# NLESC-JCER/Fortran_Davidson

Measured on AMD Instinct MI355X. Metric: Davidson iterations/sec (dense DPR solve, matrix resident in HBM) + A*V HBM GB/s vs roofline, higher is better.
Workload: dtype f64

## Files before the change

fortran_davidson_amd/csrc/engine.hip:

```cpp
#include "engine_internal.h"

thread_local std::string g_err;
int fail(const std::string& msg) {
  g_err = msg;
  return 1;
}

int bind(E* e) {
  e->h0_take = e->h0_cols;
  e->h0_cols = 0;
  HIPCHK(hipSetDevice(e->device));
  return 0;
}

int collect_events(E* e) {
  e->ev_open = 0;
  for (int i = 0; i < e->ev_used; ++i) {
    if (!e->ev_done[i]) continue;
    HIPCHK(hipEventSynchronize(e->ev[i][1]));
    float ms = 0;
    HIPCHK(hipEventElapsedTime(&ms, e->ev[i][0], e->ev[i][1]));
    if (e->ev_kind[i] == 0) {
      e->st.apply_ms += ms;
      e->st.apply_bytes += e->ev_bytes[i];
// ... 147 lines not shown

Tune tune_from_env() {
  Tune t;
  auto geti = [](const char* name, int dflt) { const char* ev = getenv(name); return ev && *ev ? atoi(ev) : dflt; };
  t.sym_wide = geti("DAV_SYM_WIDE", t.sym_wide);
  t.sym_wide32 = geti("DAV_SYM_WIDE32", t.sym_wide32);
  t.sym_pair = geti("DAV_SYM_PAIR", t.sym_pair);
  t.sym_quad = geti("DAV_SYM_QUAD", t.sym_quad);
  t.sym_overlap = geti("DAV_SYM_OVERLAP", t.sym_overlap);
  t.sym_r = geti("DAV_SYM_R", t.sym_r);
  t.sym_tall = geti("DAV_SYM_TALL", t.sym_tall);
  t.sym_gen_wide = geti("DAV_SYM_GEN_WIDE", 1);
  t.sym_run = std::max(0, geti("DAV_SYM_RUN", 0));
  t.sym_run9 = std::max(0, geti("DAV_SYM_RUN9", 0));
  t.sym_mfma4 = geti("DAV_SYM_MFMA4", t.sym_mfma4);
  t.mv_target = std::max(0, geti("DAV_MV_TARGET", 0));
  t.mv_nsplit = std::max(0, geti("DAV_MV_NSPLIT", 0));
  t.b_resident = geti("DAV_B_RESIDENT", t.b_resident);
  t.coll_direct = geti("DAV_COLL_DIRECT", t.coll_direct);
  t.pg_pin = geti("DAV_PG_PIN", t.pg_pin);
  t.gram_wgs = geti("DAV_GRAM_WGS", t.gram_wgs);
  gram_set_fuse_chunks(geti("DAV_GRAM_FUSE", 0));
  t.gjd_trace = getenv("DAV_GJD_TRACE") != nullptr;
  t.harness_libm = geti("DAV_HARNESS_LIBM", 0);
  t.no_h0 = geti("DAV_NO_H0", 0);
  t.cheb_fuse = geti("DAV_CHEB_FUSE", t.cheb_fuse);
  t.coll_select = geti("DAV_COLL_SELECT", 1);
  t.coll_trial_corrupt = geti("DAV_COLL_TRIAL_CORRUPT", 0);
  t.coll_forced = getenv("DAV_SYM_OVERLAP") != nullptr || getenv("DAV_COLL_DIRECT") != nullptr;
  return t;
// ... 263 lines not shown
    e->sm[i].host = (double*)(e->arena_host + off_smh[i]);
    HIPCHK(hipEventCreateWithFlags(&e->sm[i].done, hipEventDisableTiming));
  }
  lt.lap("carve");
  for (int i = 0; i < N_EVPAIRS; ++i) {
    HIPCHK(hipEventCreate(&e->ev[i][0]));
    HIPCHK(hipEventCreate(&e->ev[i][1]));
  }
  lt.lap("events");
  HIPCHK(hipStreamSynchronize(e->stream));
  lt.lap("memset_sync");
  lt.print("dav_create");
  return 0;
}

extern "C" int dav_destroy(dav_handle_t e) {
  if (!e) return 0;
  LapTimer lt;
  hipSetDevice(e->device);
  if (e->stream) hipStreamSynchronize(e->stream);
  if (e->comm_stream) hipStreamSynchronize(e->comm_stream);
  lt.lap("sync");
  if (e->comm && g_rccl.lib) g_rccl.CommDestroy(e->comm);
  lt.lap("comm");
  pool_begin_of_destroy();
  if (e->arena) pool_free(e->arena);
  if (e->arena_host) pool_host_free(e->arena_host);
  lt.lap("arenas");
  pool_free(e->gjd_ws);
  pool_free(e->cheb_ws);
  ingest_release(e);
  shm_release(e);
  pool_free(e->sym_slab);
  pool_free(e->rr_H); pool_free(e->rr_S); pool_free(e->rr_Y); pool_free(e->rr_theta); pool_free(e->rr_work); pool_free(e->rr_info);
  pool_free(e->rr_Ypk); pool_free(e->rr_Y2pk); pool_free(e->rr_thpk);
  lt.lap("ingest_shm_slab_rr");
  for (int i = 0; i < 2; ++i) {
    if (e->ov_packed[i]) hipEventDestroy(e->ov_packed[i]);
    if (e->ov_gathered[i]) hipEventDestroy(e->ov_gathered[i]);
    if (e->ov_reduced[i]) hipEventDestroy(e->ov_reduced[i]);
    if (e->ov_scattered[i]) hipEventDestroy(e->ov_scattered[i]);
    pool_free(e->sym_wpart2[i]);
    pool_free(e->sym_wrecv2[i]);
  }
  if (e->comm_stream) hipStreamDestroy(e->comm_stream);
  if (e->wd) {
    { std::lock_guard<std::mutex> lk(e->wd->mu); e->wd->stop = true; }
    e->wd->cv.notify_all();
    e->wd->th.join();
    for (Watchdog::Lane& l : e->wd->lane) { if (l.check.ev) hipEventDestroy(l.check.ev); if (l.latest.ev) hipEventDestroy(l.latest.ev); }
    delete e->wd;
    e->wd = nullptr;
  }
  lt.lap("overlap_watchdog");
  sym_set_release(e->sym);
  lt.lap("sym_set");
  pool_free(e->sym_wpart);
  pool_free(e->coll_stage);
  pool_free(e->cb_x);
  pool_free(e->sym_wrecv);
// ... 134 lines not shown
```

fortran_davidson_amd/csrc/engine_apply.hip:

```cpp
#include "engine_internal.h"

bool inner_f32_tiles(E* e, OpDesc& o) {
  if (e->inner_bits != 32 || o.kind != DAV_KIND_DENSE || o.storage != 1 || o.a32_refused) return false;
  if (o.a32_valid) return true;
  const size_t count = (size_t)std::max<int64_t>(e->sym.ntiles, 1) * SYM_TB * SYM_TB;
  if (!o.a32 && pool_malloc(&o.a32, sizeof(float) * count) != hipSuccess) {
    (void)hipGetLastError();
    o.a32 = nullptr;
    o.a32_refused = true;
    return false;
  }
  launch_tiles_to_f32(e->stream, o.a, o.a32, (int64_t)count);
  o.a32_valid = true;
  return true;
}

static double* sym_slab_t(const E* e, const SymLaunch& L) { return e->sym_slab + (int64_t)L.ngroups * L.dstride; }
static void sym_sweep(E* e, const SymLaunch& L, const OpDesc& o, const SymSet& set, const double* xt) {
  if (L.nitems == 0) return;
  const SymPlan* pl = L.plan;
  const void* tiles = L.use32 ? (const void*)o.a32 : (const void*)o.a;
  double *slabD = e->sym_slab, *slabT = sym_slab_t(e, L);
  const int64_t xs = e->xt_group_stride, ds = L.dstride, ts = L.tstride;
  switch (L.family) {
    case SYM_ROW_STORED:
      return launch_matvec_sym(e->stream, o.a, set.row_off, set.items, set.nitems, xt, L.kk, slabD, slabT, L.ngroups, xs, ds, ts);
    case SYM_ROW_GENERATED:
      return launch_matvec_sym_generated(e->stream, op_params(o), e->n, set.items, set.nitems, xt, L.kk, slabD, slabT, L.ngroups, xs, ds, ts);
    case SYM_SUPER:
      return launch_matvec_sym9(e->stream, L.R, o.kind != DAV_KIND_DENSE, tiles, L.use32, set.row_off, o.kind != DAV_KIND_DENSE ? op_params(o) : OpParams{},
                                e->n, e->sym_nb, pl->items, pl->nitems, pl->zslot_begin, xt, L.kk, slabD, slabT, L.nwg, xs, ds, ts, e->tune.sym_mfma4 != 0);
    case SYM_WIDE:
    case SYM_WIDE_F32:
      return launch_matvec_symw(e->stream, L.nbw, L.tall, L.use32, tiles, set.row_off, e->sym_nb, pl->items, pl->nitems, pl->zslot_begin, xt, L.kk, slabD, slabT, L.nwg, xs, ds, ts);
    case SYM_WIDE_GENERATED:
// ... 2 lines not shown
}

static void count_apply(E* e, int which, int kk) { if (which == DAV_OP_A) { e->st.applies += 1; e->st.apply_cols += kk; } }

static int pack_operand(E* e, const double* src, int kk, bool gather) {
  launch_pack_xt(e->stream, src, e->ldp, e->nloc, e->nslab, kk, e->xt, e->xt_group_stride, e->row0);
  if (!gather) return 0;
  const int ngroups = (kk + 15) / 16;
  CollGroup grp(e);
  CHK(grp.begin(5, 8.0 * (double)e->nslab * 16 * ngroups * e->nranks));
  for (int g = 0; g < ngroups; ++g)
    CHK(coll_allgather(e, e->xt + g * e->xt_group_stride + e->row0 * 16, e->xt + g * e->xt_group_stride, (size_t)e->nslab * 16));
  return grp.end("all-gather of the new block", e->stream);
}

static void sym_reduce_groups(E* e, const SymLaunch& L, const SymSet& set, const int64_t* owned, double* out, int64_t chunk_rows, bool accumulate) {
  const int64_t total_rows = (int64_t)e->nranks * e->nslab;
  const double* slabT = sym_slab_t(e, L);
  for (int g = 0; g < L.ngroups; ++g) {
    const int kg = std::min(16, L.kk - 16 * g);
    const double *d = e->sym_slab + g * L.dstride, *t = slabT + g * L.tstride;
    double* og = out + (size_t)g * 16 * (size_t)(chunk_rows ? total_rows : e->ldp);
    if (L.plan)
      launch_sym9_reduce(e->stream, d, t, L.plan->row_begin, L.plan->zslot_begin, owned, L.plan->next_owned, L.R, e->sym_nb, e->nloc, kg, og, e->ldp,
                         chunk_rows, total_rows, accumulate);
    else
      launch_sym_reduce(e->stream, d, t, set.row_begin, owned, e->sym_nb, e->nloc, kg, og, e->ldp, chunk_rows, total_rows, accumulate);
  }
}

static int ensure_sym_wpart(E* e) {
  if (e->sym_wpart) return 0;
  HIPCHK(pool_malloc(&e->sym_wpart, sizeof(double) * (size_t)e->nranks * (size_t)e->nslab * 64));
  HIPCHK(pool_malloc(&e->sym_wrecv, sizeof(double) * (size_t)e->nslab * 64));
  return 0;
}

static int sym_scatter_to_panel(E* e, int kk, double* dst, bool accumulate, const char* what, double* h0 = nullptr, size_t h0_count = 0) {
  const size_t wstride = (size_t)e->nranks * (size_t)e->nslab * 16, rstride = (size_t)e->nslab * 16;
  const int ngroups = (kk + 15) / 16;
  CollGroup grp(e);
  CHK(grp.begin(6, 8.0 * (double)e->nslab * kk * e->nranks));
  for (int g = 0; g < ngroups; ++g)
// ... 242 lines not shown
                                     "-column launch on rank " + std::to_string(e->rank) + " (DAV_SYM_QUAD=0 / DAV_SYM_PAIR=0 on every rank select narrower launches)");
      if (L.ngroups > 2) { e->sym_no_quad = true; step = 32; kk = 32; }
      else { e->sym_no_pair = true; step = 16; kk = 16; }
      L = sym_launch(e, o, set, kk, use32, L.R);
    }
    int slot = -1, kslot = -1;
    if (timed) CHK(timed_begin(e, which == DAV_OP_A ? 0 : 2, sym_stored_bytes(e, o, set, partial, use32) + 16.0 * (double)e->n * kk, &slot));
    CHK(pack_operand(e, src + (int64_t)c * e->ldp, kk, multi));
    if (timed && which == DAV_OP_A) CHK(timed_begin(e, 4, 2.0 * (double)e->n * (double)e->n * kk / e->nranks, &kslot));
    if (timed && which == DAV_OP_B) {
      const double tiles_entries = (double)set.ntiles * SYM_TB * SYM_TB;
      if (stored) CHK(timed_begin(e, 8, (use32 ? 4.0 : 8.0) * tiles_entries + 16.0 * (double)e->n * kk, &kslot));
      else CHK(timed_begin(e, 9, tiles_entries * L.gen_evals, &kslot));
      if (kslot >= 0) e->ev_flops[kslot] = 4.0 * tiles_entries * kk;
    }
    sym_sweep(e, L, o, set, e->xt);
    CHK(timed_end(e, kslot));
    sym_reduce_groups(e, L, set, owned, multi ? e->sym_wpart : dst + (int64_t)c * e->ldp, multi ? e->nslab : 0, accumulate && !multi);
    if (multi) CHK(sym_scatter_to_panel(e, kk, dst + (int64_t)c * e->ldp, accumulate, "reduce-scatter of the partial products"));
    CHK(timed_end(e, slot));
    count_apply(e, which, kk);
  }
  HIPCHK(hipGetLastError());
  return 0;
}

static void sparse_traffic(const E* e, const OpDesc& o, int k, double* bytes, double* flops) {
  const double bb = (double)o.sp.b * o.sp.b, nnz = (double)o.sp.nnz;
  *bytes = 8.0 * bb * nnz + 4.0 * nnz + 8.0 * (double)(o.sp.nrows + 1) + 8.0 * (double)e->n * k + 8.0 * (double)e->nloc * k;
  *flops = 2.0 * bb * nnz * k;
}

static int apply_identity(E* e, const double* src, int k, double* dst) { launch_copy_columns(e->stream, src, e->ldp, dst, e->ldp, e->nloc_pad, k); return 0; }
// ... 275 lines not shown
```

fortran_davidson_amd/csrc/engine_internal.h:

```cpp
#pragma once
#include "davidson_hip_private.h"
#include "kernels.h"
#include "ingest.h"

#include <dlfcn.h>
#include <fcntl.h>
#include <pthread.h>
#include <sys/mman.h>
#include <sys/stat.h>
#include <unistd.h>
#include <rccl/rccl.h>

#include <algorithm>
#include <chrono>
#include <condition_variable>
#include <ctime>
#include <mutex>
#include <cmath>
#include <cstdio>
#include <cstring>
#include <numeric>
#include <string>
#include <thread>
#include <vector>
// ... 45 lines not shown
  const char* (*GetErrorString)(ncclResult_t) = nullptr;
  ncclResult_t (*CommCount)(const ncclComm_t, int*) = nullptr;
};
extern Rccl g_rccl;
int rccl_load();
#define NCCLCHK(call)                                                                              \
  do {                                                                                             \
    ncclResult_t r_ = (call);                                                                      \
    if (r_ != ncclSuccess) return fail(std::string(#call) + " failed: " + g_rccl.GetErrorString(r_)); \
  } while (0)

struct LocalGroup;
struct ShmGroup;

struct SymPlan {
  int R = 0, nitems = 0, nsuper = 0;
  int64_t zslots = 0;
  int* items = nullptr;
  int* row_begin = nullptr;
  int* zslot_begin = nullptr;
  int* next_owned = nullptr;
};
struct SymSet {
  std::vector<int64_t> row_off_h;
  int64_t* row_off = nullptr;
  int64_t ntiles = 0;
  int nitems = 0;
  int* items = nullptr;
  int* row_begin = nullptr;
  SymPlan plan[2];
  bool built = false;
};
void sym_set_release(SymSet& s);
enum SymFamily { SYM_ROW_STORED, SYM_ROW_GENERATED, SYM_SUPER, SYM_WIDE, SYM_WIDE_GENERATED, SYM_WIDE_F32 };
struct SymLaunch {
  SymFamily family = SYM_SUPER;
  int kk = 0, ngroups = 0;
  int R = 0, nwg = 0, nbw = 1;
  bool use32 = false, tall = false;
  const SymPlan* plan = nullptr;
  int nitems = 0;
  int64_t dstride = 0, tstride = 0;
  int gen_evals = 0;
};

struct SparseStore {
  int64_t* rp = nullptr;
  int32_t* col = nullptr;
  double* val = nullptr;
  CsrItem* items = nullptr;
  CsrLong* longs = nullptr;
  double* part = nullptr;
  int nitems = 0, nlong = 0;
  int64_t nnz = 0;
  int64_t nrows = 0;
  int b = 0;
  int64_t grow0 = 0;
  uint64_t* src = nullptr;
// ... 57 lines not shown
  int sym_run = 0;
  int sym_run9 = 0;
  int sym_mfma4 = 1;
  int64_t mv_target = 0;
  int64_t mv_nsplit = 0;
  int gram_wgs = 0;
  int pg_pin = 1;
  int coll_direct = 0;
  int b_resident = 1;
  bool gjd_trace = false;
  int coll_select = 1;
  int coll_trial_corrupt = 0;
  bool coll_forced = false;
  int no_h0 = 0;
  int harness_libm = 0;
  int cheb_fuse = 1;
};
Tune tune_from_env();

enum { COLL_PATH_UNDECIDED = -1, COLL_PATH_PROGRAM_ORDER = 0, COLL_PATH_DIRECT = 1, COLL_PATH_SECOND_STREAM = 2 };
struct CollTrial {
  bool ran = false;
  int selected = COLL_PATH_PROGRAM_ORDER, columns = 0;
  double ms[3] = {0, 0, 0}, ms_max[3] = {0, 0, 0};
  bool valid[3] = {true, false, false}, valid_all[3] = {true, false, false};
  double differing[3] = {0, 0, 0}, maxdiff[3] = {0, 0, 0};
  std::string message[3];
};

enum { GUESS_NONE = 0, GUESS_ONE_SHOT = 1, GUESS_RESULT = 2 };
// ... 45 lines not shown
  std::vector<double> agree_words;
  std::vector<double> agreed_inputs;
  double* agree_pin = nullptr;
  double* h0_dev = nullptr;
  double* cb_x = nullptr;
  size_t cb_x_doubles = 0;
  double* h0_host = nullptr;
  int h0_cap = 0, h0_cols = 0, h0_take = 0;
  int h0_kind[2] = {0, 0};
  hipStream_t comm_stream = nullptr;
  bool ov_ready = false;
  hipEvent_t ov_packed[2] = {nullptr, nullptr}, ov_gathered[2] = {nullptr, nullptr}, ov_reduced[2] = {nullptr, nullptr},
             ov_scattered[2] = {nullptr, nullptr};
  double* sym_wpart2[2] = {nullptr, nullptr};
  double* sym_wrecv2[2] = {nullptr, nullptr};
  bool rr_on = false;
  int64_t rr_ld = 0;
  double *rr_H = nullptr, *rr_S = nullptr, *rr_Y = nullptr, *rr_theta = nullptr, *rr_work = nullptr, *rr_info = nullptr;
  double *rr_Ypk = nullptr, *rr_Y2pk = nullptr, *rr_thpk = nullptr;
  int64_t rr_tp = 4;
  SmallBuf sm[N_SMALL];
  size_t small_doubles = 0;
  ncclComm_t comm = nullptr;
  int comm_ranks = 0;
  LocalGroup* lg = nullptr;
  ShmGroup* shm = nullptr;
  OpDesc op[2];
  int keep_map[2] = {0, 0};
  std::vector<double> diag_host[2];
  std::vector<int64_t> basis_order;
// ... 42 lines not shown
  bool image = false;
};

int bind(E* e);
int collect_events(E* e);
int timed_begin(E* e, int kind, double bytes, int* slot);
int timed_end(E* e, int slot);
int timed_begin_on(E* e, int kind, double bytes, int* slot, hipStream_t stream);
int timed_end_on(E* e, int slot, hipStream_t stream);
int small_upload(E* e, int i, const double* src, int64_t ld, int p, int q, int64_t* ldm_out);
int small_upload_multi(E* e, int i, SmallMat* mats, int n);
int small_upload_image(E* e, int i, const double* src, int64_t ld, int p, int q, int64_t* tp_out);
double* panel_ptr(E* e, int panel, int col);
int check_panel(E* e, int panel, int c0, int k);
int create_impl(E* e, int device, int64_t n, int max_cols, int gev, int rank, int nranks);
double wall_seconds();
void watchdog_loop(Watchdog* w);
bool has_comm(E* e);
int need_comm(E* e);
bool has_test_transport(const E* e);
size_t test_transport_max_message(const E* e);
int test_allgather(E* e, const double* send, double* recv, size_t count);
int test_allreduce(E* e, double* buf, size_t count);
int test_reduce_scatter(E* e, const double* send, double* recv, size_t count);
void shm_release(E* e);
int watch_mark(E* e, const char* what, hipStream_t stream);
int coll_group_begin(E* e);
int coll_group_end(E* e, const char* what, hipStream_t stream);
void coll_group_abort(E* e);
struct CollGroup {
// ... 66 lines not shown
```

fortran_davidson_amd/csrc/engine_operators.hip:

```cpp
#include "engine_internal.h"

int refresh_diag_host(E* e, int which) {
  if (which == DAV_OP_A) e->basis_order.clear();
  std::vector<double>& d = e->diag_host[which];
  d.assign((size_t)e->n, 0.0);
  if (!has_comm(e)) {
    CHK(need_comm(e));
    HIPCHK(hipMemcpyAsync(d.data(), e->op[which].diag, sizeof(double) * e->n, hipMemcpyDeviceToHost, e->stream));
    HIPCHK(hipStreamSynchronize(e->stream));
  } else {
    CHK(coll_allgather(e, e->op[which].diag, e->gather_dev, (size_t)e->nslab));
    HIPCHK(hipMemcpyAsync(d.data(), e->gather_dev, sizeof(double) * e->n, hipMemcpyDeviceToHost, e->stream));
    HIPCHK(hipStreamSynchronize(e->stream));
  }
  return 0;
}

static bool sym_wide_enabled(const E* e) { return e->tune.sym_wide > 1; }

static int sym_schedule(const E* e, int kk, bool stored_fp64) {
  const int forced = e->tune.sym_r;
  const int nb = (int)(e->ncols_pad / SYM_TB);
  int R = nb >= 200 ? (kk <= 8 ? 4 : 2) : (nb >= 64 && stored_fp64 ? 2 : 1);
  const bool tall = stored_fp64 && kk > 8 && kk <= 16 && nb >= 200 && sym_wide_enabled(e) && e->tune.sym_tall != 0;
// ... 20 lines not shown
    L.dstride = (int64_t)set.nitems * 16 * SYM_TB;
    L.tstride = (int64_t)e->sym_nb * (e->sym_nb - 1) / 2 * 16 * SYM_TB;
  } else {
    L.plan = &set.plan[R == 4 ? 1 : 0];
    L.nitems = L.plan->nitems;
    L.dstride = (int64_t)L.nitems * R * 16 * SYM_TB;
    L.tstride = L.plan->zslots * 16 * SYM_TB;
    if (stored && !use32 && wide > 0 && ((R == 2 && (kk > 16 || wide > 1)) || (R == 4 && kk > 8 && kk <= 16))) {
      L.family = SYM_WIDE; L.nbw = kk > 16 ? 2 : 1; L.tall = R == 4;
    } else if (generated_polynomial(o) && R == 2 && kk > 16 && wide > 0 && e->tune.sym_gen_wide) {
      L.family = SYM_WIDE_GENERATED; L.nbw = 2;
    } else if (stored && use32 && wide > 1 && e->tune.sym_wide32 && R == 2 && kk <= 16) {
      L.family = SYM_WIDE_F32;
    }
    L.nwg = (L.ngroups + L.nbw - 1) / L.nbw;
  }
  L.gen_evals = stored ? 0 : L.nwg;
  return L;
}

std::vector<int> sym_group_owners(int nb, int nranks) {
  const int ng = (nb + 3) / 4;
  std::vector<int> owner(ng, 0);
  std::vector<int64_t> load(nranks, 0);
  for (int q = ng - 1; q >= 0; --q) {
    int64_t tiles = 0;
    for (int I = 4 * q; I < std::min(nb, 4 * q + 4); ++I) tiles += I + 1;
    int best = 0;
    for (int r = 1; r < nranks; ++r)
      if (load[r] < load[best]) best = r;
    owner[q] = best;
    load[best] += tiles;
  }
  return owner;
}

void sym_set_release(SymSet& s) {
  pool_free(s.row_off); pool_free(s.items); pool_free(s.row_begin);
  for (SymPlan& pl : s.plan) { pool_free(pl.items); pool_free(pl.row_begin); pool_free(pl.zslot_begin); pool_free(pl.next_owned); }
  s = SymSet();
}

int sym_setup(E* e) {
  if (e->sym.built) return 0;
  const int nb = (int)(e->ncols_pad / SYM_TB);
  e->sym_nb = nb;
  return sym_build_set(e, 0, nb, e->sym);
}

int sym_build_set(E* e, int first, int end, SymSet& out) {
  const int nb = (int)(e->ncols_pad / SYM_TB);
  sym_set_release(out);
  out.row_off_h.assign(nb, -1);
  int64_t ntiles = 0;
// ... 20 lines not shown
  std::vector<int> items;
  items.reserve(list.size() * 4 + 4);
  for (const Item& it : list) { items.push_back(it.I); items.push_back(it.J0); items.push_back(it.J1); items.push_back(it.slot); }
  items.resize(std::max<size_t>(items.size(), 4), 0);
  out.nitems = row_begin[nb];
  HIPCHK(pool_malloc(&out.items, sizeof(int) * items.size()));
  HIPCHK(pool_malloc(&out.row_begin, sizeof(int) * row_begin.size()));
  HIPCHK(hipMemcpy(out.items, items.data(), sizeof(int) * items.size(), hipMemcpyHostToDevice));
  HIPCHK(hipMemcpy(out.row_begin, row_begin.data(), sizeof(int) * row_begin.size(), hipMemcpyHostToDevice));
  for (int p = 0; p < 2; ++p) {
    SymPlan& pl = out.plan[p];
    pl.R = p == 0 ? 2 : 4;
    pl.nsuper = (nb + pl.R - 1) / pl.R;
    int64_t Cp = std::min<int64_t>(64 / pl.R, std::max<int64_t>(1, (ntiles + 3071) / (3072 * pl.R)));
    if (e->tune.sym_run9 > 0) Cp = e->tune.sym_run9;
    std::vector<Item> plist;
    std::vector<int> prow(pl.nsuper + 1, 0), zbeg(pl.nsuper + 1, 0);
    for (int S = 0; S < pl.nsuper; ++S) {
      prow[S] = (int)plist.size();
      zbeg[S + 1] = zbeg[S];
      if (!owned(S * pl.R)) continue;
      const int Imax = std::min(S * pl.R + pl.R - 1, nb - 1);
      for (int J0 = 0; J0 <= Imax; J0 += (int)Cp)
        plist.push_back({S, J0, (int)std::min<int64_t>(Imax + 1, J0 + Cp), (int)plist.size()});
      zbeg[S + 1] = zbeg[S] + Imax;
    }
    prow[pl.nsuper] = (int)plist.size();
    std::stable_sort(plist.begin(), plist.end(), [](const Item& a, const Item& b) { return a.J1 - a.J0 > b.J1 - b.J0; });
    std::vector<int> pitems;
    pitems.reserve(plist.size() * 4 + 4);
    for (const Item& it : plist) { pitems.push_back(it.I); pitems.push_back(it.J0); pitems.push_back(it.J1); pitems.push_back(it.slot); }
    pitems.resize(std::max<size_t>(pitems.size(), 4), 0);
    pl.nitems = prow[pl.nsuper];
    pl.zslots = zbeg[pl.nsuper];
    HIPCHK(pool_malloc(&pl.items, sizeof(int) * pitems.size()));
    HIPCHK(pool_malloc(&pl.row_begin, sizeof(int) * prow.size()));
    HIPCHK(pool_malloc(&pl.zslot_begin, sizeof(int) * zbeg.size()));
    HIPCHK(hipMemcpy(pl.items, pitems.data(), sizeof(int) * pitems.size(), hipMemcpyHostToDevice));
    HIPCHK(hipMemcpy(pl.row_begin, prow.data(), sizeof(int) * prow.size(), hipMemcpyHostToDevice));
    HIPCHK(hipMemcpy(pl.zslot_begin, zbeg.data(), sizeof(int) * zbeg.size(), hipMemcpyHostToDevice));
    std::vector<int> nxt(pl.nsuper + 1, pl.nsuper);
    for (int S = pl.nsuper - 1; S >= 0; --S) nxt[S] = owned(S * pl.R) ? S : nxt[S + 1];
    HIPCHK(pool_malloc(&pl.next_owned, sizeof(int) * nxt.size()));
    HIPCHK(hipMemcpy(pl.next_owned, nxt.data(), sizeof(int) * nxt.size(), hipMemcpyHostToDevice));
  }
  out.built = true;
  return 0;
}

int sym_diag(E* e, OpDesc& o) {
  if (e->nranks == 1) {
    launch_diag_sym(e->stream, o.a, e->sym.row_off, e->n, e->nloc_pad, o.diag);
    return 0;
  }
  if (!(e->comm || e->lg || e->shm)) return fail("multi-rank engine used before dav_comm_init");
  launch_diag_sym(e->stream, o.a, e->sym.row_off, e->n, e->ncols_pad, e->gather_dev);
  CHK(coll_allreduce(e, e->gather_dev, (size_t)e->ncols_pad));
  HIPCHK(hipMemcpyAsync(o.diag, e->gather_dev + e->row0, sizeof(double) * (size_t)e->nslab, hipMemcpyDeviceToDevice, e->stream));
  return 0;
}

int sym_ensure_slabs(E* e, size_t doubles) {
  if (doubles <= e->sym_slab_doubles) return 0;
  HIPCHK(hipStreamSynchronize(e->stream));
  if (e->sym_slab) HIPCHK(pool_free(e->sym_slab));
  e->sym_slab = nullptr;
  e->sym_slab_doubles = 0;
  hipError_t r = pool_malloc(&e->sym_slab, sizeof(double) * doubles);
  if (r != hipSuccess) {
    (void)hipGetLastError();
    e->sym_slab = nullptr;
    return fail("hipMalloc of the symmetric sweep slabs failed: " + std::string(hipGetErrorString(r)));
  }
  e->sym_slab_doubles = doubles;
  return 0;
}

int operator_goes(E* e, int which, bool unset) {
  OpDesc& o = e->op[which];
// ... 453 lines not shown
  CHK(bind(e));
  size_t f = 0, t = 0;
  HIPCHK(hipMemGetInfo(&f, &t));
  f += pool_idle_device_bytes(e->device);
  if (free_bytes) *free_bytes = (int64_t)f;
  if (total_bytes) *total_bytes = (int64_t)t;
  return 0;
}

extern "C" int dav_resident_fraction(dav_handle_t e, int which, double* fraction) {
  if (which < 0 || which > 1 || !fraction) return fail("dav_resident_fraction: bad arguments");
  const OpDesc& o = e->op[which];
  *fraction = (o.res_tiles > 0 && e->sym.ntiles > 0) ? (double)o.res_tiles / (double)e->sym.ntiles : 0.0;
  return 0;
}
```

fortran_davidson_amd/csrc/k_matvec_sym9.hip:

```cpp
#include "kernels.h"
#include <cstdlib>
#include <type_traits>

__device__ __forceinline__ const double* sym9_tile(const double* tiles, const int64_t* __restrict__ row_off, int I, int J) {
  return tiles + (row_off[I] + J) * (int64_t)(SYM_TB * SYM_TB);
}

__device__ __forceinline__ double mfma4_f64(double a, double b, double c) { return __builtin_amdgcn_mfma_f64_4x4x4f64(a, b, c, 0, 0, 0); }

template <int R, bool GEN, bool F32, bool M4, int HARN = 0>
__global__ __launch_bounds__(512, 1) void matvec_sym9_kernel(const void* __restrict__ tiles_v, const int64_t* __restrict__ row_off,
                                                             const int* __restrict__ items,
                                                             const int* __restrict__ zslot_begin, const double* __restrict__ xt,
                                                             double* __restrict__ slabD, double* __restrict__ slabT, int kcols,
                                                             int npair, int64_t xt_gstride, int64_t slabD_gstride,
                                                             int64_t slabT_gstride, int nb, OpParams op, int64_t n) {
  const double* tiles = static_cast<const double*>(tiles_v);
  const float* tiles32 = static_cast<const float*>(tiles_v);
  (void)tiles; (void)tiles32;
  constexpr int NCG = 4 / R;
  constexpr int NRS = 2 * R;
  constexpr int BW = 16 * NCG;
  constexpr int UPJ = SYM_TB / BW;
  constexpr int UPS = 64 / BW;
// ... 343 lines not shown
  }
#undef DAV_SYM9_LAUNCH
}

__global__ __launch_bounds__(256) void tiles_to_f32_kernel(const double* __restrict__ src, float* __restrict__ dst, int64_t count4) {
  for (int64_t e = (int64_t)blockIdx.x * 256 + threadIdx.x; e < count4; e += (int64_t)gridDim.x * 256) {
    const f64x2 a = reinterpret_cast<const f64x2*>(src)[2 * e], b = reinterpret_cast<const f64x2*>(src)[2 * e + 1];
    reinterpret_cast<float4*>(dst)[e] = float4{(float)a.x, (float)a.y, (float)b.x, (float)b.y};
  }
}
void launch_tiles_to_f32(hipStream_t st, const double* src, float* dst, int64_t count) {
  hipLaunchKernelGGL(tiles_to_f32_kernel, dim3(256 * 32), dim3(256), 0, st, src, dst, count / 4);
}

__global__ __launch_bounds__(256) void sym9_reduce_kernel(const double* __restrict__ slabD, const double* __restrict__ slabT,
                                                          const int* __restrict__ row_item_begin, const int* __restrict__ zslot_begin,
                                                          const int64_t* __restrict__ owned, const int* __restrict__ next_owned, int R, int nb,
                                                          int nsuper, int64_t nloc, int k, double* __restrict__ dst, int64_t ldd,
                                                          int64_t chunk_rows, int64_t total_rows, int accumulate) {
  const int J = blockIdx.x, col = blockIdx.y, r = threadIdx.x;
  if (col >= k) return;
  double sum = 0.0;
  const int Sown = J / R, sub = J % R;
  for (int it = row_item_begin[Sown]; it < row_item_begin[Sown + 1]; ++it)
    sum += slabD[(((int64_t)it * R + sub) * 16 + col) * SYM_TB + r];
  auto zt = [&](int S) { return slabT[(((int64_t)zslot_begin[S] + J) * 16 + col) * SYM_TB + r]; };
  double s0 = 0.0, s1 = 0.0, s2 = 0.0, s3 = 0.0;
  const int Send = (nb - 1 > J) ? nsuper : 0;
  if (!owned) {
    int S = (J + 1) / R;
    for (; S + 3 < Send; S += 4) { s0 += zt(S); s1 += zt(S + 1); s2 += zt(S + 2); s3 += zt(S + 3); }
    for (; S < Send; ++S) s0 += zt(S);
  } else {
    int S = (J + 1) / R < nsuper ? next_owned[(J + 1) / R] : nsuper;
    while (S < Send) {
      s0 += zt(S); S = next_owned[S + 1];
      if (S >= Send) break;
      s1 += zt(S); S = next_owned[S + 1];
      if (S >= Send) break;
      s2 += zt(S); S = next_owned[S + 1];
      if (S >= Send) break;
      s3 += zt(S); S = next_owned[S + 1];
    }
  }
  sum += (s0 + s1) + (s2 + s3);
  const int64_t row = (int64_t)J * SYM_TB + r;
  if (chunk_rows > 0) {
    if (row < total_rows) dst[(row / chunk_rows) * (chunk_rows * k) + (int64_t)col * chunk_rows + row % chunk_rows] = sum;
  } else {
    dst[(int64_t)col * ldd + row] = row < nloc ? (accumulate ? dst[(int64_t)col * ldd + row] + sum : sum) : 0.0;
  }
}

void launch_sym9_reduce(hipStream_t st, const double* slabD, const double* slabT, const int* row_item_begin_dev,
                        const int* zslot_begin_dev, const int64_t* owned, const int* next_owned, int R, int nb, int64_t nloc, int k, double* dst,
                        int64_t ldd, int64_t chunk_rows, int64_t total_rows, bool accumulate) {
  const int nsuper = (nb + R - 1) / R;
  hipLaunchKernelGGL(sym9_reduce_kernel, dim3(nb, k), dim3(256), 0, st, slabD, slabT, row_item_begin_dev, zslot_begin_dev, owned, next_owned, R,
                     nb, nsuper, nloc, k, dst, ldd, chunk_rows, total_rows, accumulate && chunk_rows == 0 ? 1 : 0);
}
```

fortran_davidson_amd/csrc/kernels.h:

```cpp
#pragma once
#include "common.h"

constexpr int MV_ROWS = 256;
void launch_pack_xt(hipStream_t st, const double* src, int64_t ld, int64_t nloc, int64_t nslab, int k,
                    double* xt, int64_t xt_group_stride, int64_t row_off);
void launch_matvec_dense(hipStream_t st, const double* A, int64_t lda, int64_t nrows_pad, int64_t ncols_pad,
                         const double* xt, int64_t xt_group_stride, int ngroups, double* slab,
                         int nsplit, int jc);
void launch_matvec_free(hipStream_t st, OpParams op, int64_t row0, int64_t nloc, int64_t n,
                        int64_t nrows_pad, int64_t ncols_pad, const double* xt, int64_t xt_group_stride,
                        int ngroups, double* slab, int nsplit, int jc);
void launch_slab_reduce(hipStream_t st, const double* slab, int nsplit, int64_t nrows_pad, int ngroups,
                        int64_t nloc, int k, double* dst, int64_t ldd);
size_t matvec_slab_doubles(int64_t nrows_pad, int ngroups, int nsplit);
void matvec_plan(int64_t nrows_pad, int64_t ncols_pad, int ngroups, int* nsplit, int* jc, int64_t target = 0, int64_t forced_nsplit = 0);

constexpr int GRAM_MIN_ROWS = 256;
constexpr int GRAM_FUSE_CHUNKS = 24;
constexpr int GRAM_MAX_COUNTERS = 256;
void launch_gram(hipStream_t st, const double* P, int64_t ldp, int p, const double* Q, int64_t ldq, int q,
                 int64_t nrows_pad, double* scratch, double* out_dev, unsigned* counters = nullptr, int wg_target = 0);
size_t gram_scratch_doubles(int p, int q, int64_t nrows_pad);
void gram_set_fuse_chunks(int n);
void launch_gram_multi(hipStream_t st, const double* P, int64_t ldp, int p, const double* const* Qs, int nq, int qeach, int64_t ldq,
// ... 61 lines not shown
void launch_matvec_sym_generated(hipStream_t st, OpParams op, int64_t n, const int* items_dev, int nitems, const double* xt, int kcols,
                                 double* slabD, double* slabT, int npair, int64_t xt_gstride, int64_t slabD_gstride,
                                 int64_t slabT_gstride);
void launch_sym_reduce(hipStream_t st, const double* slabD, const double* slabT, const int* row_item_begin_dev, const int64_t* owned,
                       int nb, int64_t nloc, int k, double* dst, int64_t ldd, int64_t chunk_rows, int64_t total_rows, bool accumulate = false);
void launch_matvec_sym9(hipStream_t st, int R, bool gen, const void* tiles, bool tiles_f32, const int64_t* row_off, OpParams op, int64_t n,
                        int nb, const int* items_dev, int nitems, const int* zslot_begin_dev, const double* xt, int kcols, double* slabD,
                        double* slabT, int npair, int64_t xt_gstride, int64_t slabD_gstride, int64_t slabT_gstride, bool mfma4 = true);
void launch_matvec_symw(hipStream_t st, int nbw, bool tall, bool tiles_f32, const void* tiles, const int64_t* row_off, int nb, const int* items_dev,
                        int nitems, const int* zslot_begin_dev, const double* xt, int kcols, double* slabD, double* slabT, int nwg,
                        int64_t xt_gstride, int64_t slabD_gstride, int64_t slabT_gstride);
void launch_matvec_symw_generated(hipStream_t st, OpParams op, int64_t n, int nb, const int* items_dev, int nitems, const int* zslot_begin_dev,
                                  const double* xt, int kcols, double* slabD, double* slabT, int nwg, int64_t xt_gstride, int64_t slabD_gstride,
                                  int64_t slabT_gstride);
void launch_tiles_to_f32(hipStream_t st, const double* src, float* dst, int64_t count);
void launch_sym9_reduce(hipStream_t st, const double* slabD, const double* slabT, const int* row_item_begin_dev,
                        const int* zslot_begin_dev, const int64_t* owned, const int* next_owned, int R, int nb, int64_t nloc, int k, double* dst,
                        int64_t ldd, int64_t chunk_rows, int64_t total_rows, bool accumulate = false);
void launch_generate_sym_tiles(hipStream_t st, double* tiles, const int64_t* row_off_host, int nb, int64_t n, uint64_t seed,
                               double sparsity, int use_diag, double diag_val);
void launch_retile_panel(hipStream_t st, const double* panel, int64_t ldp, int64_t nrows, int ncols, int J, int nb,
                         const int64_t* row_off, double* tiles);
void launch_diag_sym(hipStream_t st, const double* tiles, const int64_t* row_off, int64_t n, int64_t nrows, double* diag);
void launch_gather_columns_sym_rs(hipStream_t st, const double* tiles, const int64_t* row_off, int64_t n, int64_t chunk_rows,
                                  int64_t total_rows, const int64_t* idx_dev, int k, double* dst);
void launch_entries_sym(hipStream_t st, const double* tiles, const int64_t* row_off, const int64_t* idx_dev, int k, double* h0);
void launch_zero_pad_rows(hipStream_t st, double* dst, int64_t ldd, int64_t nloc, int64_t nrows_pad, int k);
void launch_entries_free(hipStream_t st, OpParams op, const int64_t* idx_dev, int k, double* h0);
void launch_entries_dense(hipStream_t st, const double* A, int64_t lda, const int64_t* idx_dev, int k, double* h0);
void launch_gather_columns_free(hipStream_t st, OpParams op, int64_t row0, int64_t nloc, int64_t nrows_pad, const int64_t* idx_dev, int k,
                                double* dst, int64_t ldd);
void launch_gather_columns_sym(hipStream_t st, const double* tiles, const int64_t* row_off, int64_t n, int64_t nrows_pad,
                               const int64_t* idx_dev, int k, double* dst, int64_t ldd);
// ... 111 lines not shown
```

Baseline: 24.20.

## Overlap symmetric matvec bands with streamed reductions; vectorize sym9 reduce kernel

Adds an optional banded schedule that splits the symmetric tile sweep into column bands across two streams. A third stream reduces each band's rows as soon as that band finishes, overlapping reduction with the remaining sweep. Separately, the sym9 reduce kernel now loads f64x2 pairs, unrolls its slab accumulation loops, and handles all column groups in a single launch instead of one launch per group. The banding adds stream/event management and plan data and is off unless DAV_SYM_BANDS is set, while the reduce-kernel change applies by default.

After: 24.21, median of 2. Within noise of the previous version (+0.1%).

```diff
diff --git a/fortran_davidson_amd/csrc/engine.hip b/fortran_davidson_amd/csrc/engine.hip
--- a/fortran_davidson_amd/csrc/engine.hip
+++ b/fortran_davidson_amd/csrc/engine.hip
@@ -185,6 +185,9 @@
   t.sym_run = std::max(0, geti("DAV_SYM_RUN", 0));
   t.sym_run9 = std::max(0, geti("DAV_SYM_RUN9", 0));
   t.sym_mfma4 = geti("DAV_SYM_MFMA4", t.sym_mfma4);
+  t.sym_bands = std::min(std::max(0, geti("DAV_SYM_BANDS", t.sym_bands)), SYM_MAX_BANDS);
+  t.sym_bands_last = geti("DAV_SYM_BANDS_LAST", t.sym_bands_last);
+  t.sym_bands_mode = geti("DAV_SYM_BANDS_MODE", t.sym_bands_mode);
   t.mv_target = std::max(0, geti("DAV_MV_TARGET", 0));
   t.mv_nsplit = std::max(0, geti("DAV_MV_NSPLIT", 0));
   t.b_resident = geti("DAV_B_RESIDENT", t.b_resident);
@@ -478,11 +481,48 @@
   return 0;
 }
 
+int sym_bands_ready(E* e) {
+  if (e->sb_ready) return 0;
+  if (e->sb_refused) return 2;
+  hipStream_t st[2] = {nullptr, nullptr};
+  hipEvent_t evs[SYM_MAX_BANDS + 2] = {};
+  int prio_least = 0, prio_greatest = 0;
+  if (hipDeviceGetStreamPriorityRange(&prio_least, &prio_greatest) != hipSuccess) { (void)hipGetLastError(); prio_greatest = 0; }
+  bool ok = hipStreamCreateWithFlags(&st[0], hipStreamNonBlocking) == hipSuccess &&
+            hipStreamCreateWithPriority(&st[1], hipStreamNonBlocking, (e->tune.sym_bands_mode & 4) ? 0 : prio_greatest) == hipSuccess;
+  for (int i = 0; ok && i < SYM_MAX_BANDS + 2; ++i) ok = hipEventCreateWithFlags(&evs[i], hipEventDisableTiming) == hipSuccess;
+  if (!ok) {
+    (void)hipGetLastError();
+    for (hipEvent_t v : evs) if (v) (void)hipEventDestroy(v);
+    for (hipStream_t s : st) if (s) (void)hipStreamDestroy(s);
+    e->sb_refused = true;
+    return 2;
+  }
+  e->sb_band_stream = st[0]; e->sb_reduce_stream = st[1];
+  e->sb_packed = evs[0]; e->sb_reduced = evs[1];
+  for (int i = 0; i < SYM_MAX_BANDS; ++i) e->sb_band[i] = evs[2 + i];
+  e->sb_ready = true;
+  return 0;
+}
+void sym_bands_release(E* e) {
+  if (e->sb_packed) hipEventDestroy(e->sb_packed);
+  if (e->sb_reduced) hipEventDestroy(e->sb_reduced);
+  for (hipEvent_t v : e->sb_band) if (v) hipEventDestroy(v);
+  if (e->sb_band_stream) hipStreamDestroy(e->sb_band_stream);
+  if (e->sb_reduce_stream) hipStreamDestroy(e->sb_reduce_stream);
+  e->sb_packed = e->sb_reduced = nullptr;
+  for (hipEvent_t& v : e->sb_band) v = nullptr;
+  e->sb_band_stream = e->sb_reduce_stream = nullptr;
+  e->sb_ready = false;
+}
+
 extern "C" int dav_destroy(dav_handle_t e) {
   if (!e) return 0;
   LapTimer lt;
   hipSetDevice(e->device);
   if (e->stream) hipStreamSynchronize(e->stream);
+  if (e->sb_band_stream) hipStreamSynchronize(e->sb_band_stream);
+  if (e->sb_reduce_stream) hipStreamSynchronize(e->sb_reduce_stream);
   if (e->comm_stream) hipStreamSynchronize(e->comm_stream);
   lt.lap("sync");
   if (e->comm && g_rccl.lib) g_rccl.CommDestroy(e->comm);
@@ -508,6 +548,7 @@
     pool_free(e->sym_wrecv2[i]);
   }
   if (e->comm_stream) hipStreamDestroy(e->comm_stream);
+  sym_bands_release(e);
   if (e->wd) {
     { std::lock_guard<std::mutex> lk(e->wd->mu); e->wd->stop = true; }
     e->wd->cv.notify_all();
diff --git a/fortran_davidson_amd/csrc/engine_apply.hip b/fortran_davidson_amd/csrc/engine_apply.hip
--- a/fortran_davidson_amd/csrc/engine_apply.hip
+++ b/fortran_davidson_amd/csrc/engine_apply.hip
@@ -16,9 +16,17 @@
 }
 
 static double* sym_slab_t(const E* e, const SymLaunch& L) { return e->sym_slab + (int64_t)L.ngroups * L.dstride; }
-static void sym_sweep(E* e, const SymLaunch& L, const OpDesc& o, const SymSet& set, const double* xt) {
+static void sym_sweep(E* e, const SymLaunch& L, const OpDesc& o, const SymSet& set, const double* xt, hipStream_t st = nullptr, int band = -1) {
   if (L.nitems == 0) return;
   const SymPlan* pl = L.plan;
+  if (!st) st = e->stream;
+  if (band >= 0) {
+    const int first = pl->band_item_begin[band], count = pl->band_item_begin[band + 1] - first;
+    if (count > 0)
+      launch_matvec_symw(st, L.nbw, L.tall, L.use32, o.a, set.row_off, e->sym_nb, pl->band_items + 4 * (int64_t)first, count, pl->zslot_begin, xt, L.kk,
+                         e->sym_slab, sym_slab_t(e, L), L.nwg, e->xt_group_stride, L.dstride, L.tstride);
+    return;
+  }
   const void* tiles = L.use32 ? (const void*)o.a32 : (const void*)o.a;
   double *slabD = e->sym_slab, *slabT = sym_slab_t(e, L);
   const int64_t xs = e->xt_group_stride, ds = L.dstride, ts = L.tstride;
@@ -51,19 +59,44 @@
   return grp.end("all-gather of the new block", e->stream);
 }
 
-static void sym_reduce_groups(E* e, const SymLaunch& L, const SymSet& set, const int64_t* owned, double* out, int64_t chunk_rows, bool accumulate) {
+static void sym_reduce_groups(E* e, const SymLaunch& L, const SymSet& set, const int64_t* owned, double* out, int64_t chunk_rows, bool accumulate,
+                              hipStream_t st = nullptr, int Jfirst = 0, int nJ = -1) {
   const int64_t total_rows = (int64_t)e->nranks * e->nslab;
   const double* slabT = sym_slab_t(e, L);
+  const int64_t ostride = 16 * (chunk_rows ? total_rows : e->ldp);
+  if (L.plan) {
+    launch_sym9_reduce(st ? st : e->stream, e->sym_slab, slabT, L.dstride, L.tstride, L.ngroups, L.plan->row_begin, L.plan->zslot_begin, owned,
+                       L.plan->next_owned, L.R, e->sym_nb, e->nloc, L.kk, Jfirst, nJ >= 0 ? nJ : e->sym_nb, out, e->ldp, ostride, chunk_rows, total_rows,
+                       accumulate);
+    return;
+  }
   for (int g = 0; g < L.ngroups; ++g) {
     const int kg = std::min(16, L.kk - 16 * g);
-    const double *d = e->sym_slab + g * L.dstride, *t = slabT + g * L.tstride;
-    double* og = out + (size_t)g * 16 * (size_t)(chunk_rows ? total_rows : e->ldp);
-    if (L.plan)
-      launch_sym9_reduce(e->stream, d, t, L.plan->row_begin, L.plan->zslot_begin, owned, L.plan->next_owned, L.R, e->sym_nb, e->nloc, kg, og, e->ldp,
-                         chunk_rows, total_rows, accumulate);
-    else
-      launch_sym_reduce(e->stream, d, t, set.row_begin, owned, e->sym_nb, e->nloc, kg, og, e->ldp, chunk_rows, total_rows, accumulate);
-  }
+    launch_sym_reduce(e->stream, e->sym_slab + g * L.dstride, slabT + g * L.tstride, set.row_begin, owned, e->sym_nb, e->nloc, kg, out + (size_t)g * ostride,
+                      e->ldp, chunk_rows, total_rows, accumulate);
+  }
+}
+
+static int sym_sweep_reduce_banded(E* e, const SymLaunch& L, const OpDesc& o, const SymSet& set, double* out, int kslot) {
+  const SymPlan* pl = L.plan;
+  hipStream_t second = e->sb_band_stream, red = e->sb_reduce_stream;
+  HIPCHK(hipEventRecord(e->sb_packed, e->stream));
+  HIPCHK(hipStreamWaitEvent(second, e->sb_packed, 0));
+  const int mode = e->tune.sym_bands_mode;
+  for (int b = 0; b < pl->nbands; ++b) {
+    hipStream_t st = (b & 1) && !(mode & 2) ? second : e->stream;
+    sym_sweep(e, L, o, set, e->xt, st, b);
+    HIPCHK(hipEventRecord(e->sb_band[b], st));
+    HIPCHK(hipStreamWaitEvent(red, e->sb_band[b], 0));
+    if (!(mode & 1)) sym_reduce_groups(e, L, set, nullptr, out, 0, false, red, pl->band_row_begin[b], pl->band_row_begin[b + 1] - pl->band_row_begin[b]);
+  }
+  if (mode & 1) sym_reduce_groups(e, L, set, nullptr, out, 0, false, red);
+  HIPCHK(hipEventRecord(e->sb_reduced, red));
+  HIPCHK(hipStreamWaitEvent(e->stream, e->sb_band[(pl->nbands - 2) | 1], 0));
+  CHK(timed_end(e, kslot));
+  HIPCHK(hipStreamWaitEvent(e->stream, e->sb_reduced, 0));
+  e->sb_applies += 1;
+  return 0;
 }
 
 static int ensure_sym_wpart(E* e) {
@@ -336,9 +369,14 @@
       else CHK(timed_begin(e, 9, tiles_entries * L.gen_evals, &kslot));
       if (kslot >= 0) e->ev_flops[kslot] = 4.0 * tiles_entries * kk;
     }
-    sym_sweep(e, L, o, set, e->xt);
-    CHK(timed_end(e, kslot));
-    sym_reduce_groups(e, L, set, owned, multi ? e->sym_wpart : dst + (int64_t)c * e->ldp, multi ? e->nslab : 0, accumulate && !multi);
+    const bool banded = L.nbands > 1 && !multi && !partial && !accumulate && sym_bands_ready(e) == 0;
+    if (banded) {
+      CHK(sym_sweep_reduce_banded(e, L, o, set, dst + (int64_t)c * e->ldp, kslot));
+    } else {
+      sym_sweep(e, L, o, set, e->xt);
+      CHK(timed_end(e, kslot));
+      sym_reduce_groups(e, L, set, owned, multi ? e->sym_wpart : dst + (int64_t)c * e->ldp, multi ? e->nslab : 0, accumulate && !multi);
+    }
     if (multi) CHK(sym_scatter_to_panel(e, kk, dst + (int64_t)c * e->ldp, accumulate, "reduce-scatter of the partial products"));
     CHK(timed_end(e, slot));
     count_apply(e, which, kk);
diff --git a/fortran_davidson_amd/csrc/engine_internal.h b/fortran_davidson_amd/csrc/engine_internal.h
--- a/fortran_davidson_amd/csrc/engine_internal.h
+++ b/fortran_davidson_amd/csrc/engine_internal.h
@@ -2,6 +2,7 @@
 #include "davidson_hip_private.h"
 #include "kernels.h"
 #include "ingest.h"
+#include "sym_bands.h"
 
 #include <dlfcn.h>
 #include <fcntl.h>
@@ -83,12 +84,16 @@
 struct ShmGroup;
 
 struct SymPlan {
-  int R = 0, nitems = 0, nsuper = 0;
+  int R = 0, nitems = 0, nsuper = 0, run = 0;
   int64_t zslots = 0;
   int* items = nullptr;
   int* row_begin = nullptr;
   int* zslot_begin = nullptr;
   int* next_owned = nullptr;
+  int nbands = 1;
+  int* band_items = nullptr;
+  int band_item_begin[SYM_MAX_BANDS + 1] = {0};
+  int band_row_begin[SYM_MAX_BANDS + 1] = {0};
 };
 struct SymSet {
   std::vector<int64_t> row_off_h;
@@ -111,6 +116,7 @@
   int nitems = 0;
   int64_t dstride = 0, tstride = 0;
   int gen_evals = 0;
+  int nbands = 1;
 };
 
 struct SparseStore {
@@ -198,6 +204,9 @@
   bool coll_forced = false;
   int no_h0 = 0;
   int harness_libm = 0;
+  int sym_bands = 0;
+  int sym_bands_last = 100;
+  int sym_bands_mode = 0;
   int cheb_fuse = 1;
 };
 Tune tune_from_env();
@@ -273,6 +282,10 @@
              ov_scattered[2] = {nullptr, nullptr};
   double* sym_wpart2[2] = {nullptr, nullptr};
   double* sym_wrecv2[2] = {nullptr, nullptr};
+  hipStream_t sb_band_stream = nullptr, sb_reduce_stream = nullptr;
+  hipEvent_t sb_packed = nullptr, sb_reduced = nullptr, sb_band[SYM_MAX_BANDS] = {};
+  bool sb_ready = false, sb_refused = false;
+  int64_t sb_applies = 0;
   bool rr_on = false;
   int64_t rr_ld = 0;
   double *rr_H = nullptr, *rr_S = nullptr, *rr_Y = nullptr, *rr_theta = nullptr, *rr_work = nullptr, *rr_info = nullptr;
@@ -345,6 +358,8 @@
 double* panel_ptr(E* e, int panel, int col);
 int check_panel(E* e, int panel, int c0, int k);
 int create_impl(E* e, int device, int64_t n, int max_cols, int gev, int rank, int nranks);
+int sym_bands_ready(E* e);
+void sym_bands_release(E* e);
 double wall_seconds();
 void watchdog_loop(Watchdog* w);
 bool has_comm(E* e);
diff --git a/fortran_davidson_amd/csrc/engine_operators.hip b/fortran_davidson_amd/csrc/engine_operators.hip
--- a/fortran_davidson_amd/csrc/engine_operators.hip
+++ b/fortran_davidson_amd/csrc/engine_operators.hip
@@ -58,6 +58,7 @@
       L.family = SYM_WIDE_F32;
     }
     L.nwg = (L.ngroups + L.nbw - 1) / L.nbw;
+    if (L.family == SYM_WIDE && L.nbw == 2 && !L.tall && e->nranks == 1) L.nbands = L.plan->nbands;
   }
   L.gen_evals = stored ? 0 : L.nwg;
   return L;
@@ -81,7 +82,7 @@
 
 void sym_set_release(SymSet& s) {
   pool_free(s.row_off); pool_free(s.items); pool_free(s.row_begin);
-  for (SymPlan& pl : s.plan) { pool_free(pl.items); pool_free(pl.row_begin); pool_free(pl.zslot_begin); pool_free(pl.next_owned); }
+  for (SymPlan& pl : s.plan) { pool_free(pl.items); pool_free(pl.row_begin); pool_free(pl.zslot_begin); pool_free(pl.next_owned); pool_free(pl.band_items); }
   s = SymSet();
 }
 
@@ -132,6 +133,7 @@
     pl.nsuper = (nb + pl.R - 1) / pl.R;
     int64_t Cp = std::min<int64_t>(64 / pl.R, std::max<int64_t>(1, (ntiles + 3071) / (3072 * pl.R)));
     if (e->tune.sym_run9 > 0) Cp = e->tune.sym_run9;
+    pl.run = (int)Cp;
     std::vector<Item> plist;
     std::vector<int> prow(pl.nsuper + 1, 0), zbeg(pl.nsuper + 1, 0);
     for (int S = 0; S < pl.nsuper; ++S) {
@@ -161,6 +163,23 @@
     for (int S = pl.nsuper - 1; S >= 0; --S) nxt[S] = owned(S * pl.R) ? S : nxt[S + 1];
     HIPCHK(pool_malloc(&pl.next_owned, sizeof(int) * nxt.size()));
     HIPCHK(hipMemcpy(pl.next_owned, nxt.data(), sizeof(int) * nxt.size(), hipMemcpyHostToDevice));
+    const int want = std::max(1, e->tune.sym_bands);
+    if (pl.R == 2 && e->nranks == 1 && first == 0 && end >= nb && want > 1) {
+      int jb[SYM_MAX_BANDS + 1];
+      pl.nbands = sym_band_partition(nb, pl.R, (int)Cp, want, e->tune.sym_bands_last, jb, pl.band_row_begin);
+      auto band_of = [&](const Item& it) { int b = 0; while (it.J0 >= jb[b + 1]) ++b; return b; };
+      std::vector<Item> blist = plist;
+      std::stable_sort(blist.begin(), blist.end(), [&](const Item& a, const Item& b) { return band_of(a) < band_of(b); });
+      std::vector<int> bitems;
+      bitems.reserve(blist.size() * 4 + 4);
+      pl.band_item_begin[0] = 0;
+      for (int b = 0; b < pl.nbands; ++b)
+        pl.band_item_begin[b + 1] = pl.band_item_begin[b] + (int)std::count_if(blist.begin(), blist.end(), [&](const Item& it) { return band_of(it) == b; });
+      for (const Item& it : blist) { bitems.push_back(it.I); bitems.push_back(it.J0); bitems.push_back(it.J1); bitems.push_back(it.slot); }
+      bitems.resize(std::max<size_t>(bitems.size(), 4), 0);
+      HIPCHK(pool_malloc(&pl.band_items, sizeof(int) * bitems.size()));
+      HIPCHK(hipMemcpy(pl.band_items, bitems.data(), sizeof(int) * bitems.size(), hipMemcpyHostToDevice));
+    }
   }
   out.built = true;
   return 0;
@@ -181,6 +200,8 @@
 int sym_ensure_slabs(E* e, size_t doubles) {
   if (doubles <= e->sym_slab_doubles) return 0;
   HIPCHK(hipStreamSynchronize(e->stream));
+  if (e->sb_band_stream) HIPCHK(hipStreamSynchronize(e->sb_band_stream));
+  if (e->sb_reduce_stream) HIPCHK(hipStreamSynchronize(e->sb_reduce_stream));
   if (e->sym_slab) HIPCHK(pool_free(e->sym_slab));
   e->sym_slab = nullptr;
   e->sym_slab_doubles = 0;
@@ -664,3 +685,16 @@
   *fraction = (o.res_tiles > 0 && e->sym.ntiles > 0) ? (double)o.res_tiles / (double)e->sym.ntiles : 0.0;
   return 0;
 }
+
+extern "C" __attribute__((visibility("default"))) int symband_partition(int nb, int R, int Cp, int B, int last_percent, int* jb, int* rb) {
+  if (nb < 1 || (R != 2 && R != 4) || !jb || !rb) return -1;
+  return sym_band_partition(nb, R, Cp, B, last_percent, jb, rb);
+}
+extern "C" __attribute__((visibility("default"))) int symband_engine_info(dav_handle_t e, int* nbands, int* run, int64_t* banded_launches) {
+  if (!e || !e->sym.built) return -1;
+  const SymPlan& pl = e->sym.plan[0];
+  if (nbands) *nbands = pl.nbands;
+  if (run) *run = pl.run;
+  if (banded_launches) *banded_launches = e->sb_applies;
+  return 0;
+}
diff --git a/fortran_davidson_amd/csrc/k_matvec_sym9.hip b/fortran_davidson_amd/csrc/k_matvec_sym9.hip
--- a/fortran_davidson_amd/csrc/k_matvec_sym9.hip
+++ b/fortran_davidson_amd/csrc/k_matvec_sym9.hip
@@ -1,4 +1,5 @@
 #include "kernels.h"
+#include <algorithm>
 #include <cstdlib>
 #include <type_traits>
 
@@ -381,22 +382,46 @@
 }
 
 __global__ __launch_bounds__(256) void sym9_reduce_kernel(const double* __restrict__ slabD, const double* __restrict__ slabT,
+                                                          int64_t slabD_gstride, int64_t slabT_gstride,
                                                           const int* __restrict__ row_item_begin, const int* __restrict__ zslot_begin,
                                                           const int64_t* __restrict__ owned, const int* __restrict__ next_owned, int R, int nb,
-                                                          int nsuper, int64_t nloc, int k, double* __restrict__ dst, int64_t ldd,
-                                                          int64_t chunk_rows, int64_t total_rows, int accumulate) {
-  const int J = blockIdx.x, col = blockIdx.y, r = threadIdx.x;
+                                                          int nsuper, int64_t nloc, int kcols, int Jfirst, double* __restrict__ dst, int64_t ldd,
+                                                          int64_t dst_gstride, int64_t chunk_rows, int64_t total_rows, int accumulate) {
+  const int J = Jfirst + blockIdx.x, grp = blockIdx.z;
+  const int col = 2 * blockIdx.y + (threadIdx.x >> 7), r = 2 * (threadIdx.x & 127);
+  const int k = kcols - 16 * grp < 16 ? kcols - 16 * grp : 16;
   if (col >= k) return;
-  double sum = 0.0;
+  slabD += grp * slabD_gstride;
+  slabT += grp * slabT_gstride;
+  dst += grp * dst_gstride;
+  f64x2 sum = f64x2{0.0, 0.0};
   const int Sown = J / R, sub = J % R;
-  for (int it = row_item_begin[Sown]; it < row_item_begin[Sown + 1]; ++it)
-    sum += slabD[(((int64_t)it * R + sub) * 16 + col) * SYM_TB + r];
-  auto zt = [&](int S) { return slabT[(((int64_t)zslot_begin[S] + J) * 16 + col) * SYM_TB + r]; };
-  double s0 = 0.0, s1 = 0.0, s2 = 0.0, s3 = 0.0;
+  auto dt = [&](int it) { return *reinterpret_cast<const f64x2*>(slabD + (((int64_t)it * R + sub) * 16 + col) * SYM_TB + r); };
+  {
+    int it = row_item_begin[Sown];
+    const int itend = row_item_begin[Sown + 1];
+    for (; it + 3 < itend; it += 4) {
+      const f64x2 d0 = dt(it), d1 = dt(it + 1), d2 = dt(it + 2), d3 = dt(it + 3);
+      sum += d0; sum += d1; sum += d2; sum += d3;
+    }
+    for (; it < itend; ++it) sum += dt(it);
+  }
+  auto zt = [&](int S) { return *reinterpret_cast<const f64x2*>(slabT + (((int64_t)zslot_begin[S] + J) * 16 + col) * SYM_TB + r); };
+  f64x2 s0 = f64x2{0.0, 0.0}, s1 = s0, s2 = s0, s3 = s0;
   const int Send = (nb - 1 > J) ? nsuper : 0;
   if (!owned) {
     int S = (J + 1) / R;
-    for (; S + 3 < Send; S += 4) { s0 += zt(S); s1 += zt(S + 1); s2 += zt(S + 2); s3 += zt(S + 3); }
+    for (; S + 7 < Send; S += 8) {
+      f64x2 v[8];
+#pragma unroll
+      for (int u = 0; u < 8; ++u) v[u] = zt(S + u);
+      s0 += v[0]; s1 += v[1]; s2 += v[2]; s3 += v[3];
+      s0 += v[4]; s1 += v[5]; s2 += v[6]; s3 += v[7];
+    }
+    for (; S + 3 < Send; S += 4) {
+      const f64x2 v0 = zt(S), v1 = zt(S + 1), v2 = zt(S + 2), v3 = zt(S + 3);
+      s0 += v0; s1 += v1; s2 += v2; s3 += v3;
+    }
     for (; S < Send; ++S) s0 += zt(S);
   } else {
     int S = (J + 1) / R < nsuper ? next_owned[(J + 1) / R] : nsuper;
@@ -411,18 +436,25 @@
     }
   }
   sum += (s0 + s1) + (s2 + s3);
-  const int64_t row = (int64_t)J * SYM_TB + r;
-  if (chunk_rows > 0) {
-    if (row < total_rows) dst[(row / chunk_rows) * (chunk_rows * k) + (int64_t)col * chunk_rows + row % chunk_rows] = sum;
-  } else {
-    dst[(int64_t)col * ldd + row] = row < nloc ? (accumulate ? dst[(int64_t)col * ldd + row] + sum : sum) : 0.0;
-  }
-}
-
-void launch_sym9_reduce(hipStream_t st, const double* slabD, const double* slabT, const int* row_item_begin_dev,
-                        const int* zslot_begin_dev, const int64_t* owned, const int* next_owned, int R, int nb, int64_t nloc, int k, double* dst,
-                        int64_t ldd, int64_t chunk_rows, int64_t total_rows, bool accumulate) {
+#pragma unroll
+  for (int h = 0; h < 2; ++h) {
+    const int64_t row = (int64_t)J * SYM_TB + r + h;
+    const double v = h == 0 ? sum.x : sum.y;
+    if (chunk_rows > 0) {
+      if (row < total_rows) dst[(row / chunk_rows) * (chunk_rows * k) + (int64_t)col * chunk_rows + row % chunk_rows] = v;
+    } else {
+      dst[(int64_t)col * ldd + row] = row < nloc ? (accumulate ? dst[(int64_t)col * ldd + row] + v : v) : 0.0;
+    }
+  }
+}
+
+void launch_sym9_reduce(hipStream_t st, const double* slabD, const double* slabT, int64_t slabD_gstride, int64_t slabT_gstride, int ngroups,
+                        const int* row_item_begin_dev, const int* zslot_begin_dev, const int64_t* owned, const int* next_owned, int R, int nb,
+                        int64_t nloc, int kcols, int Jfirst, int nJ, double* dst, int64_t ldd, int64_t dst_gstride, int64_t chunk_rows,
+                        int64_t total_rows, bool accumulate) {
+  if (nJ <= 0 || ngroups <= 0) return;
   const int nsuper = (nb + R - 1) / R;
-  hipLaunchKernelGGL(sym9_reduce_kernel, dim3(nb, k), dim3(256), 0, st, slabD, slabT, row_item_begin_dev, zslot_begin_dev, owned, next_owned, R,
-                     nb, nsuper, nloc, k, dst, ldd, chunk_rows, total_rows, accumulate && chunk_rows == 0 ? 1 : 0);
-}
+  hipLaunchKernelGGL(sym9_reduce_kernel, dim3(nJ, (std::min(kcols, 16) + 1) / 2, ngroups), dim3(256), 0, st, slabD, slabT, slabD_gstride,
+                     slabT_gstride, row_item_begin_dev, zslot_begin_dev, owned, next_owned, R, nb, nsuper, nloc, kcols, Jfirst, dst, ldd, dst_gstride,
+                     chunk_rows, total_rows, accumulate && chunk_rows == 0 ? 1 : 0);
+}
diff --git a/fortran_davidson_amd/csrc/kernels.h b/fortran_davidson_amd/csrc/kernels.h
--- a/fortran_davidson_amd/csrc/kernels.h
+++ b/fortran_davidson_amd/csrc/kernels.h
@@ -99,9 +99,10 @@
                                   const double* xt, int kcols, double* slabD, double* slabT, int nwg, int64_t xt_gstride, int64_t slabD_gstride,
                                   int64_t slabT_gstride);
 void launch_tiles_to_f32(hipStream_t st, const double* src, float* dst, int64_t count);
-void launch_sym9_reduce(hipStream_t st, const double* slabD, const double* slabT, const int* row_item_begin_dev,
-                        const int* zslot_begin_dev, const int64_t* owned, const int* next_owned, int R, int nb, int64_t nloc, int k, double* dst,
-                        int64_t ldd, int64_t chunk_rows, int64_t total_rows, bool accumulate = false);
+void launch_sym9_reduce(hipStream_t st, const double* slabD, const double* slabT, int64_t slabD_gstride, int64_t slabT_gstride, int ngroups,
+                        const int* row_item_begin_dev, const int* zslot_begin_dev, const int64_t* owned, const int* next_owned, int R, int nb,
+                        int64_t nloc, int kcols, int Jfirst, int nJ, double* dst, int64_t ldd, int64_t dst_gstride, int64_t chunk_rows,
+                        int64_t total_rows, bool accumulate = false);
 void launch_generate_sym_tiles(hipStream_t st, double* tiles, const int64_t* row_off_host, int nb, int64_t n, uint64_t seed,
                                double sparsity, int use_diag, double diag_val);
 void launch_retile_panel(hipStream_t st, const double* panel, int64_t ldp, int64_t nrows, int ncols, int J, int nb,
diff --git a/fortran_davidson_amd/csrc/sym_bands.h b/fortran_davidson_amd/csrc/sym_bands.h
--- /dev/null
+++ b/fortran_davidson_amd/csrc/sym_bands.h
@@ -0,0 +1,24 @@
+#pragma once
+#include <cstdint>
+
+constexpr int SYM_MAX_BANDS = 16;
+
+inline int sym_band_partition(int nb, int R, int Cp, int B, int last_percent, int* jb, int* rb) {
+  if (B < 1) B = 1;
+  if (B > SYM_MAX_BANDS) B = SYM_MAX_BANDS;
+  if (Cp < 1) Cp = 1;
+  if (last_percent < 1 || last_percent > 100) last_percent = 100;
+  const int64_t total = (int64_t)nb * (nb + 1) / 2;
+  const int64_t shares = 100 * (int64_t)(B - 1) + last_percent;
+  int nbands = 0;
+  jb[0] = 0;
+  for (int J = Cp; J < nb && nbands + 1 < B; J += Cp) {
+    const int64_t before = (int64_t)J * nb - (int64_t)J * (J - 1) / 2;
+    if (before * shares >= total * 100 * (int64_t)(nbands + 1)) jb[++nbands] = J;
+  }
+  jb[++nbands] = nb;
+  rb[0] = 0;
+  for (int b = 1; b < nbands; ++b) rb[b] = R * (jb[b] / R);
+  rb[nbands] = nb;
+  return nbands;
+}
```
